# yhw-yhw/TalkSHOW

Hardware: AMD Instinct MI355X
Metric: generated SMPL-X frames/sec (10 s @ 30 fps clips), whole job (higher is better)
Workload: dtype f32; 1 GPU; BASELINE configs[1]: batch=32 x 10 s clips, body+hand VQ-VAE encode -> PixelCNN greedy decode -> VQ decode, 30 fps; batch_per_gpu=32, frames_per_clip=300, coalesce=8, streams=3

## Files before the change

include/talkshow_hip_debug.h:

```cpp
#ifndef TALKSHOW_HIP_DEBUG_H
#define TALKSHOW_HIP_DEBUG_H

#include "talkshow_hip.h"

#ifdef __cplusplus
extern "C" {
#endif

int ts_stream_create_cus(ts_ctx *ctx, int cu_first, int cu_count, void **out_stream);
int ts_debug_skinny_trace(unsigned long long *out, int max_records);
int ts_debug_clock_sample(unsigned long long *dev_out, int n, int window_us, void *stream);
int ts_debug_conv_bands(int M, int N, int groups, int *out4);
int ts_debug_split_tile(int bid, int MT, int NT, int gw, int *out2);
int ts_debug_tile_weights(const float *W, int N, int K, long ldw, int epi, int gateD, float *out);

int ts_op_conv1d_timed(ts_ctx *ctx, const float *x_dev, int B, int Lin, int Cin, const float *w_packed_dev,
                       const float *bias_dev, int Cout, int K, int tile, int iters, float *out_dev, float *ms_out,
                       void *stream);
int ts_op_conv1d_strided_timed(ts_ctx *ctx, const float *x_dev, int B, int Lin, int Cin, const float *w_packed_dev,
                               const float *bias_dev, int Cout, int K, int stride, int tile, int iters, float *out_dev,
                               float *ms_out, void *stream);

int ts_op_conv_taps48_timed(ts_ctx *ctx, const float *x_dev, int B, int T, int G, int ntap, const float *w_dev, const float *bias_dev,
                            const float *res_dev, int iters, float *out_dev, float *ms_out, void *stream);
// ... 118 lines not shown
int ts_debug_code_tables_plan(int V, int D, int B, int r, int j, int last_row, const char *knob_list, int64_t *out12);
int ts_debug_pixelcnn_tables(ts_pixelcnn *pix, int mode);
int64_t ts_debug_pixelcnn_work(ts_pixelcnn *pix, void *stream, int which, float *buf_dev, int64_t cap_floats, int put);
int ts_debug_code_table_stage(ts_pixelcnn *pix, int which, const int32_t *tok_dev, int B, const float *add1, const float *add2, const float *cls,
                              float *pre, float *out, float *q1, float *q0, void *stream);

int ts_debug_mixed_plan(const int32_t *hrows, int B, int max_counts, int32_t *active_out);

int ts_debug_rep_table(const ts_repeat *rep_host, int n_rep, int B, int V, int32_t *words_out);

int ts_op_vq_argmin_pair_masked(ts_ctx *ctx, const float *z_body_dev, const float *z_hand_dev, const int32_t *lens_dev, int B, int H_max,
                                const float *codebook_body_dev, const float *codebook_hand_dev, int ncode_body, int ncode_hand, int dim_body,
                                int dim_hand, int64_t *codes_dev, void *stream);
int ts_debug_vq_argmin_pair_masked(ts_ctx *ctx, const float *z_body_dev, const float *z_hand_dev, const int32_t *lens_dev, int B, int H_max,
                                   const float *codebook_body_dev, const float *codebook_hand_dev, int ncode_body, int ncode_hand,
                                   int dim_body, int dim_hand, int64_t *codes_dev, int form, int iters, void *stream);

int ts_debug_wino_lowering(int cin, int cout, int k, int stride, const char *knob_list, int B, int L, int *out5);
int ts_debug_wino_weights(const float *w, int cout, int cin, float *out);
int ts_debug_wino_transform(ts_ctx *ctx, int which, int nnet, int B, int L, int C, int act, const int32_t *lens_dev, int shr, int shl,
                            const void *const *ptrs, void *stream);
int ts_debug_wino_gemm(ts_ctx *ctx, int nnet, const float *V0, const float *V1, const float *U0, const float *U1, float *O0, float *O1, int M,
                       int C, void *stream);

int ts_debug_body_stream_plan(const int64_t *state4, int t, int flush, int enc_lowered, int64_t *out14);
int ts_debug_stream_stage_mfcc(const float *tail, const float *chunk, float *win, float *next, int B, int n_tail, int t, int cap, int Tw,
                               int next0, int n_next, void *stream);
int ts_debug_stream_emit(const int64_t *codes, int64_t *ring, int64_t *lat_body, int64_t *lat_hand, int B, int n, int A, int RC, int v0, int Hw,
                         void *stream);
int ts_debug_stream_keep_rows(const float *src, float *dst, int B, int R, int r0, int n, int W, void *stream);

int ts_debug_gather_rows(const float *table, int ld_table, int nrows, const int64_t *idx, long idx_stride, int M, int width, float *out,
                         int ldo, int L, const int32_t *lens, int len_shr, void *stream);
int ts_debug_pad_rows(const float *src, int lds, int c, float *dst, int ldd, int cpad, int B, int L, const int32_t *lens, void *stream);
int ts_debug_mask_rows(int64_t *codes, float *logprob, int B, int H, const int32_t *lens, void *stream);
int ts_debug_iota_i64(int64_t *dst, int n, int64_t first, void *stream);
int ts_debug_i64_to_i32(const int64_t *src, int32_t *dst, long n, void *stream);
int ts_debug_set_words3(uint64_t *dst, uint64_t a, uint64_t b, uint64_t c, void *stream);
int ts_debug_row_sqnorm(const float *e, int n, int dim, float *out, void *stream);

int ts_debug_skinny_chain(ts_ctx *ctx, int M, int K, int gate, int iters, int debug, float *us_out);

#ifdef __cplusplus
}
#endif
#endif
// ... 1 lines not shown
```

talkshow_amd/_lib.py:

```python
import ctypes as C
import os

import numpy as np
import torch

_HERE = os.path.dirname(os.path.abspath(__file__))
LIB_PATH = os.environ.get("TS_LIB_PATH") or os.path.join(_HERE, "lib", "libtalkshow_hip.so")

TS_SAMPLE_GREEDY, TS_SAMPLE_UNIFORMS, TS_SAMPLE_PHILOX, TS_TEACHER_FORCED = 0, 1, 2, 3


class TsTensor(C.Structure):
    _fields_ = [("name", C.c_char_p), ("data", C.POINTER(C.c_float)), ("ndim", C.c_int32), ("shape", C.c_int64 * 4)]


_vp, _i, _i64, _u64, _fp = C.c_void_p, C.c_int, C.c_int64, C.c_uint64, C.POINTER(C.c_float)


class TsSampling(C.Structure):
    _fields_ = [("temperature", C.c_float), ("top_p", C.c_float), ("top_k", C.c_int32), ("reserved", C.c_int32)]


_sp = C.POINTER(TsSampling)

# ... 154 lines not shown
    "ts_pixelcnn_generate_mixed": (_i, [_vp, _vp, _vp, C.POINTER(C.c_int32), _vp, _i, _i, _i, _vp, _u64, _vp, _vp, _vp]),
    "ts_vqvae_decode_pair_masked": (_i, [_vp, _vp, _vp, _vp, _vp, _i, _i, _vp, _vp]),
    "ts_debug_mixed_plan": (_i, [C.POINTER(C.c_int32), _i, _i, C.POINTER(C.c_int32)]),
    "ts_body_vq_infer": (_i, [_vp, _vp, _vp, _i, _i, _vp, _vp, _vp]),
    "ts_op_conv1d": (_i, [_vp, _vp, _i, _i, _i, _fp, _fp, _i, _i, _i, _i, _i, _i, _vp, _vp]),
    "ts_op_conv1d_timed": (_i, [_vp, _vp, _i, _i, _i, _vp, _vp, _i, _i, _i, _i, _vp, C.POINTER(C.c_float), _vp]),
    "ts_op_conv_taps48_timed": (_i, [_vp, _vp, _i, _i, _i, _i, _vp, _vp, _vp, _i, _vp, C.POINTER(C.c_float), _vp]),
    "ts_op_conv1d_strided_timed": (_i, [_vp, _vp, _i, _i, _i, _vp, _vp, _i, _i, _i, _i, _i, _vp, C.POINTER(C.c_float), _vp]),
    "ts_debug_pixelcnn_graphs": (_i, [_vp, _vp]),
    "ts_debug_code_tables_plan": (_i, [_i, _i, _i, _i, _i, _i, C.c_char_p, C.POINTER(_i64)]),
    "ts_debug_pixelcnn_tables": (_i, [_vp, _i]),
    "ts_debug_pixelcnn_work": (_i64, [_vp, _vp, _i, _vp, _i64, _i]),
    "ts_debug_code_table_stage": (_i, [_vp, _i, _vp, _i, _vp, _vp, _vp, _vp, _vp, _vp, _vp, _vp]),
    "ts_debug_conv_run": (_i, [_vp, C.POINTER(ConvProblem), _i, C.c_char_p, _i, C.POINTER(_i), _vp]),
    "ts_debug_conv_sk_plan": (_i, [_i, _i, _i, _i, C.POINTER(C.c_int)]),
    "ts_debug_conv_sk_run": (_i, [_i, _i, _i, _i, C.POINTER(C.c_int)]),
    "ts_debug_conv_sk_supported": (_i, []),
    "ts_pixelcnn_graph_captures": (C.c_long, [_vp, _vp]),
    "ts_pixelcnn_prepare": (_i, [_vp, _i, _i, _i, _vp]),
    "ts_debug_wino_lowering": (_i, [_i, _i, _i, _i, C.c_char_p, _i, _i, C.POINTER(_i)]),
    "ts_debug_wino_weights": (_i, [_vp, _i, _i, _vp]),
    "ts_debug_wino_transform": (_i, [_vp, _i, _i, _i, _i, _i, _i, _vp, _i, _i, C.POINTER(_vp), _vp]),
    "ts_debug_wino_gemm": (_i, [_vp, _i, _vp, _vp, _vp, _vp, _vp, _vp, _i, _i, _vp]),
    "ts_debug_conv_plan": (_i, [_i, _i, _i, _i, _i, C.POINTER(_i), _i, _i, C.c_char_p, C.POINTER(_i)]),
    "ts_debug_skinny_plan": (_i, [C.POINTER(_i), _i, C.c_char_p, C.POINTER(_i)]),
    "ts_debug_skinny_run": (_i, [_vp, C.POINTER(SkinnyProblem), _i, C.c_char_p, C.POINTER(_i), _vp]),
    "ts_debug_gate_act": (_i, [_vp, _vp, _vp, C.c_long, _vp]),
    "ts_debug_gelu": (_i, [_vp, _vp, C.c_long, _vp]),
    "ts_debug_attention": (_i, [_vp, _i, _i, _i, _i, C.c_float, _vp, _vp]),
    "ts_debug_layernorm_rows": (_i, [_vp, _i, C.c_long, _i, _vp, _vp, _vp, _i, _i, _vp, _i, _vp]),
    "ts_debug_lerp_ln": (_i, [_vp, _i, _i, _i, _vp, _vp, _vp, _vp]),
    "ts_debug_w2v_conv0": (_i, [_vp, _i, _i, _vp, _vp, _vp, _i, _vp, _vp]),
    "ts_debug_fill_id": (_i, [_vp, _i, _vp, _vp, _i, _vp, _i, _i, _i, _i, _vp]),
    "ts_debug_attention_mixed": (_i, [_vp, C.POINTER(C.c_int32), _vp, _i, _i, _i, _i, C.c_float, _vp, _vp]),
    "ts_debug_layernorm_rows_lens": (_i, [_vp, _i, _i, _i, _vp, _i, _vp, _vp, _vp, _i, _i, _vp, _i, _vp]),
    "ts_debug_lerp_ln_lens": (_i, [_vp, _i, _i, _i, _vp, _vp, _vp, _vp, _vp, _vp]),
    "ts_debug_w2v_conv0_lens": (_i, [_vp, _i, _i, _vp, _vp, _vp, _vp, _i, _vp, _vp]),
    "ts_debug_fill_id_lens": (_i, [_vp, _i, _vp, _vp, _i, _vp, _i, _i, _i, _i, _vp, _vp]),
    "ts_debug_face_mixed_grid": (_i, [C.POINTER(C.c_int32), _i, _i, C.POINTER(C.c_int32), _i]),
    "ts_debug_face_packed_layout": (_i, [C.POINTER(C.c_int32), C.POINTER(C.c_int32), _i, C.POINTER(_i64), C.POINTER(_i64), C.POINTER(_i64)]),
    "ts_debug_face_generate_mixed": (_i, [_vp, _vp, C.POINTER(C.c_int32), _vp, C.POINTER(C.c_int32), _vp, _i, _i, _i, _vp, _vp, _vp, _vp, _i]),
    "ts_debug_attention_packed": (_i, [_vp, C.POINTER(C.c_int32), _vp, _i, _i, _i, C.c_float, _vp, _vp]),
    "ts_debug_pack_rows": (_i, [_vp, C.POINTER(C.c_int32), _i, _i, _i, _vp, _vp]),
    "ts_debug_unpack_rows": (_i, [_vp, C.POINTER(C.c_int32), _vp, _i, _i, _i, _vp, _vp]),
    "ts_debug_w2v_conv0_packed": (_i, [_vp, _i, _i, C.POINTER(C.c_int32), _vp, _vp, _vp, _vp, _i, _vp, _vp]),
    "ts_debug_lerp_ln_packed": (_i, [_vp, _i, _i, C.POINTER(C.c_int32), _vp, _vp, _vp, _vp, _vp, _vp]),
# ... 605 lines not shown
```

talkshow_amd/csrc/api.cpp:

```cpp
#include <cstring>
#include <vector>
#include "host_common.h"
#include "conv_tile.h"
#include "skinny_desc.h"

using namespace ts;

namespace {
struct BodyWork {
    DevBuf feat;
    DevBuf lat[2];
    DevBuf given;
};
BodyWork &body_work(hipStream_t s) {
    static StreamWorks<BodyWork> works;
    return works.get(s);
}
}

namespace ts {
template <class Get>
static Knobs read_knobs(Get get) {
    Knobs v;
    auto num = [&](const char *name, int dflt) { const char *e = get(name); return e && e[0] ? std::atoi(e) : dflt; };
    v.conv_bands = num("TS_CONV_BANDS", 1) != 0;
    v.conv_ring = num("TS_CONV_RING", 9);
    v.conv_deal = num("TS_CONV_DEAL", 1) != 0;
    v.conv_ring_paired = num("TS_CONV_RING_PAIRED", 1) != 0;
    v.conv_taps48 = num("TS_CONV_TAPS48", 1) != 0;
    v.face_pack = num("TS_FACE_PACK", 0) != 0;
    v.conv_sk = num("TS_CONV_SK", 1);
    v.conv_wino = num("TS_CONV_WINO", -1);
    v.w2v_moments = num("TS_W2V_MOMENTS", 1) != 0;
    v.vq_lds = num("TS_VQ_LDS", 1) != 0;
    v.vq_pair = num("TS_VQ_PAIR", 1) != 0;
    v.split_xcd = num("TS_SPLIT_XCD", 8);
    v.prof_log = num("TS_PROF_LOG", 0) != 0;
    if (const char *e = get("TS_NO_GRAPH")) v.no_graph = e[0] && e[0] != '0';
    v.pix_defer_p = num("TS_PIX_DEFER_P", -1);
    v.pix_tables = num("TS_PIX_TABLES", -1);
    v.skinny_v = num("TS_SKINNY_V", 1);
    v.skinny_nt = num("TS_SKINNY_NT", 16);
    v.skinny_tiled = num("TS_SKINNY_TILED", 1) != 0;
    v.wide_min = num("TS_SKINNY_WIDE_MIN", 160);
    v.skinny_shape = num("TS_SKINNY_SHAPE", 0);
    v.skinny_trace = num("TS_SKINNY_TRACE", 0);
    v.wide_ablate = num("TS_SKINNY_WIDE_ABLATE", 0);
    v.wide_pair = num("TS_SKINNY_WIDE_PAIR", 1) != 0;
    return v;
}
const Knobs &knobs() {
    static const Knobs k = read_knobs([](const char *name) { return std::getenv(name); });
    return k;
}
static Knobs knobs_from_list(const char *list) {
// ... 1176 lines not shown
    std::memset(&w, 0, sizeof(w));
    w.nnet = nnet;
    w.B = B, w.L = L, w.J = (L + 3) / 4, w.C = C, w.act = act;
    w.lens = lens_dev, w.len_shr = shr, w.len_shl = shl;
    for (int i = 0; i < nnet; ++i) {
        const void *const *q = ptrs + 6 * i;
        w.x[i] = (const float *)q[0], w.V[i] = (float *)q[1], w.O[i] = (const float *)q[2], w.bias[i] = (const float *)q[3];
        w.res[i] = (const float *)q[4], w.y[i] = (float *)q[5];
    }
    MiscScope ms(ctx, (hipStream_t)stream);
    TS_HIP(ts::launch_wino(which, w, (hipStream_t)stream));
    return 0;
}

int ts_debug_wino_gemm(ts_ctx *ctx, int nnet, const float *V0, const float *V1, const float *U0, const float *U1, float *O0, float *O1, int M,
                       int C, void *stream) {
    if (!ctx || nnet < 1 || nnet > 2 || !V0 || !U0 || !O0 || (nnet == 2 && (!V1 || !U1 || !O1)) || M < 1 || C < 32 || C % 32)
        return fail("ts_debug_wino_gemm: bad argument");
    const float *V[2] = {V0, V1}, *U[2] = {U0, U1};
    float *O[2] = {O0, O1};
    return ts::run_wino_gemm(ctx, nnet, V, U, O, M, C, round_up(C, 128), (hipStream_t)stream);
}

int ts_debug_gather_rows(const float *table, int ld_table, int nrows, const int64_t *idx, long idx_stride, int M, int width, float *out,
                         int ldo, int L, const int32_t *lens, int len_shr, void *stream) {
    if (!table || !idx || !out || M < 1 || width < 1) return fail("ts_debug_gather_rows: bad argument");
    if (!lens && L == 0) TS_HIP(ts::launch_gather_rows(table, ld_table, nrows, idx, idx_stride, M, width, out, ldo, (hipStream_t)stream));
    else TS_HIP(ts::launch_gather_rows_masked(table, ld_table, nrows, idx, idx_stride, M, width, out, ldo, L, lens, len_shr, (hipStream_t)stream));
    return 0;
}
int ts_debug_pad_rows(const float *src, int lds, int c, float *dst, int ldd, int cpad, int B, int L, const int32_t *lens, void *stream) {
    if (!src || !dst || B < 1 || L < 1 || cpad < 1) return fail("ts_debug_pad_rows: bad argument");
    if (!lens) TS_HIP(ts::launch_pad_rows(src, lds, c, dst, ldd, cpad, (long)B * L, (hipStream_t)stream));
    else TS_HIP(ts::launch_pad_rows_masked(src, lds, c, dst, ldd, cpad, B, L, lens, (hipStream_t)stream));
    return 0;
}
int ts_debug_mask_rows(int64_t *codes, float *logprob, int B, int H, const int32_t *lens, void *stream) {
    if ((!codes && !logprob) || !lens || B < 1 || H < 1) return fail("ts_debug_mask_rows: bad argument");
    if (codes) TS_HIP(ts::launch_mask_codes(codes, B, H, lens, (hipStream_t)stream));
    if (logprob) TS_HIP(ts::launch_mask_logprob(logprob, B, H, lens, (hipStream_t)stream));
    return 0;
}
int ts_debug_iota_i64(int64_t *dst, int n, int64_t first, void *stream) {
    if (!dst || n < 1) return fail("ts_debug_iota_i64: bad argument");
    TS_HIP(ts::launch_iota_i64(dst, n, first, (hipStream_t)stream));
    return 0;
// ... 19 lines not shown
```

talkshow_amd/csrc/conv_wino.hip:

```cpp
#include "kernels.h"
#include "conv_tile.h"

namespace ts {

namespace {

__device__ __forceinline__ f32x4 ld4(const float *p) { return *reinterpret_cast<const f32x4 *>(p); }
__device__ __forceinline__ void st4(float *p, f32x4 v) { *reinterpret_cast<f32x4 *>(p) = v; }

__device__ __forceinline__ void wino_bt(const f32x4 (&d)[6], f32x4 (&v)[6]) {
#pragma clang fp contract(off)
    v[0] = (4.f * d[0] - 5.f * d[2]) + d[4];
    v[1] = ((d[3] - 4.f * d[1]) - 4.f * d[2]) + d[4];
    v[2] = ((4.f * d[1] - 4.f * d[2]) - d[3]) + d[4];
    v[3] = ((2.f * d[3] - 2.f * d[1]) - d[2]) + d[4];
    v[4] = ((2.f * d[1] - d[2]) - 2.f * d[3]) + d[4];
    v[5] = (4.f * d[1] - 5.f * d[3]) + d[5];
}

__device__ __forceinline__ f32x4 wino_at_row(const f32x4 (&m)[6], const int r) {
#pragma clang fp contract(off)
    if (r == 0) return (((m[0] + m[1]) + m[2]) + m[3]) + m[4];
    if (r == 1) return ((m[1] - m[2]) + 2.f * m[3]) - 2.f * m[4];
    if (r == 2) return ((m[1] + m[2]) + 4.f * m[3]) + 4.f * m[4];
// ... 3 lines not shown
__device__ __forceinline__ f32x4 wino_finish(f32x4 y, const f32x4 bias, const float *res, const int act) {
#pragma clang fp contract(off)
    f32x4 v = y + bias;
    if (res) v = v + ld4(res);
#pragma unroll
    for (int q = 0; q < 4; ++q) {
        float e = v[q];
        if (act == 1) e = e >= 0.f ? e : e * 0.2f;
        else if (act == 2) e = e > 0.f ? e : 0.f;
        else if (act == 3) e = gelu_fast(e);
        v[q] = e;
    }
    return v;
}

struct WinoItem {
    int net, b, j, c, Lb;
    long row;
    bool ok;
};
__device__ __forceinline__ WinoItem wino_item(const WinoParams &p) {
    WinoItem w;
    const int c4 = p.C >> 2;
    const long idx = (long)blockIdx.x * blockDim.x + threadIdx.x;
    w.net = blockIdx.y;
    w.row = idx / c4;
    w.c = (int)(idx - w.row * c4) << 2;
    w.ok = w.row < (long)p.B * p.J;
    w.b = (int)(w.row / p.J);
    w.j = (int)(w.row - (long)w.b * p.J);
    w.Lb = p.L;
    if (w.ok && p.lens) {
        const int l = (p.lens[w.b] >> p.len_shr) << p.len_shl;
        w.Lb = l < p.L ? l : p.L;
    }
    return w;
}

__device__ __forceinline__ void wino_load_tile(const float *O, const long comp_stride, const long row, const int C, const int c, f32x4 (&m)[6]) {
#pragma unroll
    for (int i = 0; i < 6; ++i) m[i] = ld4(O + i * comp_stride + row * C + c);
}

__global__ __launch_bounds__(256) void wino_in_kernel(const WinoParams p) {
    const WinoItem w = wino_item(p);
    if (!w.ok) return;
    const float *x = p.x[w.net] + (long)w.b * p.L * p.C + w.c;
    f32x4 d[6], v[6];
// ... 35 lines not shown
    const float *O = p.O[w.net];
    const f32x4 bias = ld4(p.bias[w.net] + w.c);
    const f32x4 zero{0.f, 0.f, 0.f, 0.f};
    f32x4 m[6], d[6], v[6];
    d[0] = zero;
    if (w.j > 0 && 4 * w.j - 1 < w.Lb) {
        wino_load_tile(O, cs, w.row - 1, p.C, w.c, m);
        d[0] = wino_finish(wino_at_row(m, 3), bias, nullptr, p.act);
    }
    wino_load_tile(O, cs, w.row, p.C, w.c, m);
#pragma unroll
    for (int r = 0; r < 4; ++r) d[1 + r] = 4 * w.j + r < w.Lb ? wino_finish(wino_at_row(m, r), bias, nullptr, p.act) : zero;
    d[5] = zero;
    if (w.j + 1 < p.J && 4 * w.j + 4 < w.Lb) {
        wino_load_tile(O, cs, w.row + 1, p.C, w.c, m);
        d[5] = wino_finish(wino_at_row(m, 0), bias, nullptr, p.act);
    }
    wino_bt(d, v);
    float *V = p.V[w.net] + w.row * p.C + w.c;
#pragma unroll
    for (int i = 0; i < 6; ++i) st4(V + i * cs, v[i]);
}

}

hipError_t launch_wino(int which, const WinoParams &p, hipStream_t stream) {
    if (p.nnet < 1 || p.nnet > 2 || p.B < 1 || p.L < 1 || p.C < 4 || (p.C & 3) || p.J != (p.L + 3) / 4 || p.act < 0 || p.act > 3 ||
        (p.lens && (p.len_shr < 0 || p.len_shl < 0)))
        return hipErrorInvalidValue;
    const long items = (long)p.B * p.J * (p.C >> 2);
    if (items + 255 >= (1l << 31)) return hipErrorInvalidValue;
    for (int n = 0; n < p.nnet; ++n) {
        const bool in = which == 0 ? p.x[n] && p.V[n] : which == 1 ? p.O[n] && p.bias[n] && p.y[n] : p.O[n] && p.bias[n] && p.V[n];
        if (!in) return hipErrorInvalidValue;
    }
    const dim3 grid((unsigned)((items + 255) / 256), p.nnet);
    if (which == 0) hipLaunchKernelGGL(wino_in_kernel, grid, dim3(256), 0, stream, p);
    else if (which == 1) hipLaunchKernelGGL(wino_out_kernel, grid, dim3(256), 0, stream, p);
    else if (which == 2) hipLaunchKernelGGL(wino_out_in_kernel, grid, dim3(256), 0, stream, p);
    else return hipErrorInvalidValue;
    return hipGetLastError();
}

void wino_transform_weights(const float *w, int cout, int cin, int npad, float *out) {
    static const double G[6][3] = {{1.0 / 4, 0, 0},          {-1.0 / 6, -1.0 / 6, -1.0 / 6}, {-1.0 / 6, 1.0 / 6, -1.0 / 6},
                                   {1.0 / 24, 1.0 / 12, 1.0 / 6}, {1.0 / 24, -1.0 / 12, 1.0 / 6}, {0, 0, 1}};
    for (int i = 0; i < 6; ++i)
        for (int o = 0; o < npad; ++o)
            for (int c = 0; c < cin; ++c) {
                double u = 0.0;
                if (o < cout) {
                    const float *g = w + ((size_t)o * cin + c) * 3;
                    u = G[i][0] * (double)g[0] + G[i][1] * (double)g[1] + G[i][2] * (double)g[2];
                }
                out[((size_t)i * npad + o) * cin + c] = (float)u;
            }
}

}
```

talkshow_amd/csrc/host_common.h:

```cpp
#pragma once
#include <hip/hip_runtime.h>

#include <cmath>
#include <cstring>
#include <map>
#include <atomic>
#include <memory>
#include <mutex>
#include <string>
#include <vector>

#include "../../include/talkshow_hip.h"
#include "../../include/talkshow_hip_debug.h"
#include "kernels.h"

namespace ts {

void set_error(const std::string &m);
inline int fail(const std::string &m) {
    set_error(m);
    return 1;
}

#define TS_HIP(expr)                                                                              \
// ... 173 lines not shown
};

struct ConvLayer {
    int kind = 0;
    int cin = 0, cin_pad = 0, cout = 0, cout_pad = 0, npad = 0, ktot = 0;
    int act = 0;
    int ngroups = 1, nseg = 0;
    ConvSeg segs[2][4];
    DevBuf w, bias;
    DevBuf wp;
    DevBuf wino;
    std::string name;
};

int pack_conv_layer(const StateDict &sd, const std::string &conv_key, const std::string &norm_key,
                    const std::string &res_key, int kind, int k, int cin, int cout, int act, ConvLayer *out);
int pack_linear_layer(const float *w, long ldw, const float *bias, int N, int K, ConvLayer *out);

int pack_conv_raw(const float *w, const float *bias, int cout, int cin, int K, const int *taps, int act, ConvLayer *out);

int conv_layer_params(const ConvLayer &layer, const float *x, int ldx, int B, int Lin, const float *res, int ldr,
                      float *out, int ldo, int out_col0, int n_store, ConvParams *p);

int run_wino_gemm(ts_ctx *ctx, int n, const float *const *V, const float *const *U, float *const *O, int M, int c, int npad, hipStream_t s);

int convnet_hidden(const ts_convnet *n);
int face_mixed_grid(const int32_t *frames, int B, int heads, std::vector<int> &work);
struct FacePacked {
    std::vector<int> feat_off, row0;
    long feat_rows = 0, rows = 0;
    int len[7] = {};
};
constexpr int FACE_FC_K[6] = {3, 3, 3, 3, 2, 2};
int face_packed_layout(const int32_t *ns, const int32_t *frames, int B, FacePacked *out);
int vqvae_in_dim(const ts_vqvae *v);
int vq_encode_pair_masked(ts_vqvae *vb, ts_vqvae *vh, const float *poses, int poses_ld, const int32_t *lens_dev, int B, int T_max, int64_t *codes,
                          int codes_H, float *z_body, float *z_hand, int form, hipStream_t s);

struct MixedPass {
    const int64_t *ids;
    const int32_t *lens_host, *lens_dev;
    int B, rows, mode;
    const float *uniforms;
    uint64_t seed;
    const int64_t *clip_index;
    int64_t *codes;
};
// ... 45 lines not shown
```

talkshow_amd/csrc/kernels.h:

```cpp
#pragma once
#include <hip/hip_runtime.h>
#include <stdint.h>

namespace ts {

struct Knobs;

struct ConvSeg {
    int d;
    int c0;
    int len;
    int ntap;
};

struct ConvGroup {
    const float *x;
    const float *w;
    const float *bias;
    const float *res;
    float *out;
    int out_col0;
    int nseg;
    ConvSeg seg[4];
};
// ... 89 lines not shown
    return true;
}

hipError_t launch_split_weight_planes(const float *w, float *planes, long rows, int K, hipStream_t stream);
double conv_gemm_flops(const ConvParams &p);

constexpr int WINO_MIN_C = 512;
inline bool wino_lowered(int kind, int k, int cin, int cout, int knob) {
    const bool geom = kind == 0 && k == 3 && cin == cout && cin % 32 == 0;
    return geom && knob != 0 && (knob == 1 || cout >= WINO_MIN_C);
}
struct WinoParams {
    int nnet;
    int B, L, J, C;
    int act;
    const int *lens;
    int len_shr, len_shl;
    const float *x[2];
    float *V[2];
    const float *O[2];
    const float *bias[2];
    const float *res[2];
    float *y[2];
};
hipError_t launch_wino(int which, const WinoParams &p, hipStream_t stream);
void wino_transform_weights(const float *w, int cout, int cin, int npad, float *out);

struct SkinnySeg {
    const float *base;
    const int *gidx;
    long row_stride;
    long gidx_stride;
    int row_shift;
    int len;
    int tiled_w;
};

enum { EPI_LINEAR = 0, EPI_GATE = 1 };
constexpr int SKINNY_MAX_SEG = 3;
constexpr int SKINNY_MAX_PROBLEMS = 6;

struct SkinnyParams {
    int M, N;
    int nseg, Ktot;
    SkinnySeg seg[SKINNY_MAX_SEG];
    const float *W;
// ... 126 lines not shown
    bool vq_lds = true;
    bool vq_pair = true;
    int conv_ring = 9;
    bool w2v_moments = true;
    int conv_sk = 1;
    bool face_pack = false;
    bool conv_taps48 = true;
    bool conv_ring_paired = true;
    bool conv_deal = true;
    int split_xcd = 8;
    bool prof_log = false;
    bool no_graph = false;
    int pix_defer_p = -1;
    int pix_tables = -1;
    int skinny_v = 1;
    int skinny_nt = 16;
    bool skinny_tiled = true;
    int wide_min = 160;
    int skinny_shape = 0;
    int skinny_trace = 0;
    bool wide_pair = true;
    int wide_ablate = 0;
    int conv_wino = -1;
};
const Knobs &knobs();

constexpr size_t CODE_TABLE_CAP_BYTES = (size_t)192 << 20;
constexpr int CODE_TABLE_MIN_CLIPS = 64;
struct CodeTablePlan {
    bool fits = false;
    int waves_v0 = 0, sets_v0 = 0, waves_hg = 0;
    size_t bytes_v0 = 0, bytes_hg = 0;
};
inline CodeTablePlan code_table_plan(int V, int D, const Knobs &k) {
    CodeTablePlan t;
    if (V < 1 || D < 32 || D % 32) return t;
    t.waves_v0 = code_table_waves(2 * D);
    t.sets_v0 = 1 + t.waves_v0 / 2;
    t.waves_hg = code_table_waves(D);
    t.bytes_v0 = (size_t)3 * t.sets_v0 * V * 4 * D * sizeof(float);
    t.bytes_hg = (size_t)V * 2 * D * sizeof(float);
    t.fits = k.skinny_nt != 32 && (size_t)V * 4 * D * sizeof(float) * 15 <= CODE_TABLE_CAP_BYTES;
    return t;
}
inline bool code_table_pass(bool built, int mode, int B) { return built && (mode > 0 || (mode < 0 && B >= CODE_TABLE_MIN_CLIPS)); }
inline bool code_table_v0_row(int r) { return r >= 1; }
// ... 178 lines not shown
```

talkshow_amd/csrc/models.cpp:

```cpp
#include <algorithm>
#include <cstdio>
#include "host_common.h"
#include "conv_tile.h"

namespace ts {

static thread_local std::string g_err;
void set_error(const std::string &m) { g_err = m; }
const char *last_error() { return g_err.c_str(); }

namespace {
std::mutex &scoped_mu() {
    static std::mutex m;
    return m;
}
std::vector<StreamScoped *> &scoped_all() {
    static std::vector<StreamScoped *> v;
    return v;
}
}
StreamScoped::StreamScoped() {
    std::lock_guard<std::mutex> g(scoped_mu());
    scoped_all().push_back(this);
}
// ... 242 lines not shown

int pack_linear_layer(const float *w, long ldw, const float *bias, int N, int K, ConvLayer *L) {
    L->kind = 0;
    L->cin = K;
    L->cin_pad = round_up(K, 32);
    L->cout = N;
    L->cout_pad = round_up(N, 32);
    L->npad = round_up(N, 128);
    L->act = 0;
    L->ngroups = 1;
    L->nseg = 1;
    L->ktot = L->cin_pad;
    L->segs[0][0] = ConvSeg{0, 0, L->cin_pad};
    std::vector<float> wp((size_t)L->npad * L->ktot, 0.f), bp(L->npad, 0.f);
    for (int o = 0; o < N; ++o) {
        for (int i = 0; i < K; ++i) wp[(size_t)o * L->ktot + i] = w[(long)o * ldw + i];
        if (bias) bp[o] = bias[o];
    }
    TS_TRY(L->w.upload(wp.data(), wp.size() * sizeof(float)));
    TS_TRY(L->bias.upload(bp.data(), bp.size() * sizeof(float)));
    return 0;
}

int run_wino_gemm(ts_ctx *ctx, int n, const float *const *V, const float *const *U, float *const *O, int M, int c, int npad, hipStream_t s) {
    auto dist = [](const float *a, const float *b) { return (long)((reinterpret_cast<intptr_t>(a) - reinterpret_cast<intptr_t>(b)) / (intptr_t)sizeof(float)); };
    ConvParams p;
    std::memset(&p, 0, sizeof(p));
    p.M = p.Lout = p.Lin = M;
    p.stride = 1;
    p.ldx = p.ldo = c;
    p.N = c;
    p.Ktot = c;
    p.ngroups = 6 * n;
    p.zdiv = 6;
    ConvGroup &g = p.g[0];
    g.x = V[0];
    g.w = U[0];
    g.out = O[0];
    g.nseg = 1;
    g.seg[0] = ConvSeg{0, 0, c, 1};
    p.x_zs1 = p.o_zs1 = (long)M * c;
    p.w_zs1 = (long)npad * c;
    if (n == 2) {
        p.x_zs0 = dist(V[1], V[0]);
        p.o_zs0 = dist(O[1], O[0]);
        p.w_zs0 = dist(U[1], U[0]);
    }
    const ConvPlan pl = plan_conv(p, 0, knobs(), false);
    const bool ring = pl.engine == ConvEngine::Reg && pl.bm == 128 && pl.bn == 128 && knobs().conv_ring > 0 && conv_gemm_ring_takes(p);
    return run_conv(ctx, p, ring ? 35 : 0, s);
}

int conv_layer_params(const ConvLayer &L, const float *x, int ldx, int B, int Lin, const float *res, int ldr,
                      float *out, int ldo, int out_col0, int n_store, ConvParams *p) {
    std::memset(p, 0, sizeof(*p));
    const int Lrows = L.kind == 1 ? Lin / 2 : Lin;
    p->M = B * Lrows;
    p->Lout = Lrows;
    p->Lin = Lin;
    p->stride = L.kind == 1 ? 2 : 1;
    p->ldx = ldx;
    p->ldr = ldr;
    p->N = n_store;
    p->Ktot = L.ktot;
// ... 116 lines not shown
                2 * L[0]->ngroups <= 4;
    if (same) {
        ConvParams &q = p[0];
        for (int g = 0; g < L[1]->ngroups; ++g) q.g[q.ngroups + g] = p[1].g[g];
        q.ngroups += L[1]->ngroups;
        return run_conv(ctx, q, 0, s);
    }
    for (int i = 0; i < n; ++i) TS_TRY(run_conv(ctx, p[i], 0, s));
    return 0;
}

int run_layer(ts_ctx *ctx, const ConvLayer &L, const float *x, int ldx, int B, int Lin, const float *res, int ldr,
              float *out, int ldo, int col0, int nstore, hipStream_t s, int *Lout, const LenMask *mk = nullptr) {
    const ConvLayer *Lp[1] = {&L};
    const float *xp[1] = {x}, *rp[1] = {res};
    float *op[1] = {out};
    return run_layer_n(ctx, 1, Lp, xp, ldx, B, Lin, rp, ldr, op, ldo, &col0, &nstore, s, Lout, mk);
}

size_t stack_wino_floats(const Stack &st, int c, int B, int L) {
    return st.tail.wino.p ? (size_t)6 * round_up(B * ((L + 3) / 4), 128) * c : 0;
}

int run_stack_wino(ts_ctx *ctx, int n, const Stack *const *st, Pool *const *pool, int cur, int c, int B, int L, hipStream_t s, int *out_idx,
                   const LenMask *mk) {
    WinoParams w;
    std::memset(&w, 0, sizeof(w));
    w.nnet = n;
    w.B = B, w.L = L, w.J = (L + 3) / 4, w.C = c;
    if (mk) w.lens = mk->lens, w.len_shr = mk->shr, w.len_shl = mk->shl;
    const int o = pool[0]->pick(cur), M = B * w.J;
    for (int i = 0; i < n; ++i) {
        if (pool[i]->wv.bytes < (size_t)6 * M * c * sizeof(float) || pool[i]->wo.bytes < (size_t)6 * M * c * sizeof(float))
            return fail("run_stack_wino: the Winograd arenas were not grown for this pass");
        w.x[i] = pool[i]->buf(cur);
        w.V[i] = pool[i]->wv.f();
        w.O[i] = pool[i]->wo.f();
        w.res[i] = pool[i]->buf(cur);
        w.y[i] = pool[i]->buf(o);
    }
    const ConvLayer *Lp[2];
    {
        MiscScope ms(ctx, s);
        TS_HIP(launch_wino(0, w, s));
    }
    const size_t nl = st[0]->layers.size();
    for (size_t k = 0; k <= nl; ++k) {
        for (int i = 0; i < n; ++i) {
            Lp[i] = k < nl ? st[i]->layers[k].get() : &st[i]->tail;
            w.bias[i] = Lp[i]->bias.f();
        }
        w.act = Lp[0]->act;
        const float *Vp[2] = {w.V[0], w.V[1]}, *Up[2] = {Lp[0]->wino.f(), n == 2 ? Lp[1]->wino.f() : nullptr};
        float *Op[2] = {pool[0]->wo.f(), n == 2 ? pool[1]->wo.f() : nullptr};
        TS_TRY(run_wino_gemm(ctx, n, Vp, Up, Op, M, c, Lp[0]->npad, s));
        MiscScope ms(ctx, s);
        TS_HIP(launch_wino(k < nl ? 2 : 1, w, s));
    }
    *out_idx = o;
    return 0;
}

int run_stack_n(ts_ctx *ctx, int n, const Stack *const *st, Pool *const *pool, int cur, int c, int B, int L, hipStream_t s,
                int *out_idx, const LenMask *mk = nullptr) {
    bool wino = true;
    for (int i = 0; i < n; ++i) {
        wino = wino && st[i]->tail.wino.p;
        for (const auto &l : st[i]->layers) wino = wino && l->wino.p;
    }
    if (wino) return run_stack_wino(ctx, n, st, pool, cur, c, B, L, s, out_idx, mk);
    int h = cur, tmp = 0;
    const int ns[2] = {c, c};
    const ConvLayer *Lp[2];
    const float *xp[2], *rp[2];
    float *op[2];
    for (size_t k = 0; k < st[0]->layers.size(); ++k) {
        const int o = pool[0]->pick(cur, h);
        for (int i = 0; i < n; ++i) { Lp[i] = st[i]->layers[k].get(); xp[i] = pool[i]->buf(h); op[i] = pool[i]->buf(o); }
        TS_TRY(run_layer_n(ctx, n, Lp, xp, c, B, L, nullptr, 0, op, c, nullptr, ns, s, &tmp, mk));
        h = o;
    }
    const int o = pool[0]->pick(cur, h);
    for (int i = 0; i < n; ++i) { Lp[i] = &st[i]->tail; xp[i] = pool[i]->buf(h); rp[i] = pool[i]->buf(cur); op[i] = pool[i]->buf(o); }
    TS_TRY(run_layer_n(ctx, n, Lp, xp, c, B, L, rp, c, op, c, nullptr, ns, s, &tmp, mk));
    *out_idx = o;
    return 0;
}

int run_trunk_n(int n, ts_convnet *const *net, const float *const *x, int x_ld, int B, int T, hipStream_t s, int *out_idx,
                int *H, const int *lens = nullptr) {
    if (T < 4) return fail("sequence too short: need T >= 4 frames");
    LenMask m0{lens, 0, 0}, m1{lens, 1, 0}, m2{lens, 2, 0};
    const LenMask *k0 = lens ? &m0 : nullptr, *k1 = lens ? &m1 : nullptr, *k2 = lens ? &m2 : nullptr;
// ... 47 lines not shown
    TS_TRY(run_layer_n(ctx, n, Lp, xp, hid / 2, B, L, nullptr, 0, op, hid, nullptr, ns, s, &L, k2));
    cur = o;
    for (int i = 0; i < n; ++i) Sp[i] = &net[i]->s3;
    TS_TRY(run_stack_n(ctx, n, Sp, pool, cur, hid, B, L, s, &o, k2));
    *out_idx = o;
    *H = L;
    return 0;
}

int run_trunk(ts_convnet *n, const float *x, int x_ld, int B, int T, hipStream_t s, int *out_idx, int *H, const int *lens = nullptr) {
    ts_convnet *np[1] = {n};
    const float *xp[1] = {x};
    return run_trunk_n(1, np, xp, x_ld, B, T, s, out_idx, H, lens);
}

}

struct ts_vqvae {
    ts_ctx *ctx = nullptr;
    int in_dim = 0, emb = 0, ncode = 0, hid = 0, nres = 0;
    ts_convnet enc;
    DevBuf codebook, code_sq;
    DevBuf aft_table;
    ConvLayer aft;
    Stack d1, d2, d3;
    ConvLayer up2, up3, project;
    struct Work {
        Pool pool;
        DevBuf z, lat;
        DevBuf pair;
    };
    StreamWorks<Work> works;
    Work &work(hipStream_t s) { return works.get(s); }
};

namespace {

int vq_encode_n(int n, ts_vqvae *const *vq, const float *const *poses, int poses_ld, int B, int T, float *const *z_out,
                int64_t *const *lat_out, float *const *q_out, hipStream_t s, int *Hout) {
    ts_ctx *ctx = vq[0]->ctx;
    int idx = 0, H = 0, tmp = 0;
    ts_convnet *nets[2];
    for (int i = 0; i < n; ++i) nets[i] = &vq[i]->enc;
    TS_TRY(run_trunk_n(n, nets, poses, poses_ld, B, T, s, &idx, &H));
    const ConvLayer *Lp[2];
    const float *xp[2];
// ... 42 lines not shown
    for (int i = 0; i < n; ++i) {
        if (vq[i]->hid != hid) return fail("paired VQ-VAEs must have the same width");
        pool[i] = &vq[i]->work(s).pool;
        TS_TRY(pool[i]->ensure((size_t)B * H * hid));
        TS_TRY(pool[i]->ensure_wino(std::max({stack_wino_floats(vq[i]->d1, hid, B, H), stack_wino_floats(vq[i]->d2, hid / 2, B, 2 * H),
                                              stack_wino_floats(vq[i]->d3, hid / 4, B, 4 * H)})));
        if (z && z[i]) {
            int tmp = 0;
            TS_TRY(run_layer(ctx, vq[i]->aft, z[i], vq[i]->emb, B, H, nullptr, 0, pool[i]->buf(0), hid, 0, hid, s, &tmp));
        } else {
            if (vq[i]->ncode == 0) return fail("this network has no codebook (auto-encoder): decode continuous latents");
            MiscScope ms(ctx, s);
            if (lens) TS_HIP(launch_gather_rows_masked(vq[i]->aft_table.f(), hid, vq[i]->ncode, lat[i], 1, B * H, hid, pool[i]->buf(0), hid, H, lens, 2, s));
            else TS_HIP(launch_gather_rows(vq[i]->aft_table.f(), hid, vq[i]->ncode, lat[i], 1, B * H, hid, pool[i]->buf(0), hid, s));
        }
    }
    int cur = 0, o = 0, L = H;
    const ConvLayer *Lp[2];
    const Stack *Sp[2];
    const float *xp[2];
    float *op[2];
    int ns[2];
    for (int i = 0; i < n; ++i) Sp[i] = &vq[i]->d1;
    TS_TRY(run_stack_n(ctx, n, Sp, pool, cur, hid, B, L, s, &o, k0));
    cur = o;
    o = pool[0]->pick(cur);
    for (int i = 0; i < n; ++i) { Lp[i] = &vq[i]->up2; xp[i] = pool[i]->buf(cur); op[i] = pool[i]->buf(o); ns[i] = hid / 2; }
    TS_TRY(run_layer_n(ctx, n, Lp, xp, hid, B, L, nullptr, 0, op, hid / 2, nullptr, ns, s, &L, k0));
    cur = o;
    for (int i = 0; i < n; ++i) Sp[i] = &vq[i]->d2;
    TS_TRY(run_stack_n(ctx, n, Sp, pool, cur, hid / 2, B, L, s, &o, k1));
    cur = o;
    o = pool[0]->pick(cur);
    for (int i = 0; i < n; ++i) { Lp[i] = &vq[i]->up3; xp[i] = pool[i]->buf(cur); op[i] = pool[i]->buf(o); ns[i] = hid / 4; }
    TS_TRY(run_layer_n(ctx, n, Lp, xp, hid / 2, B, L, nullptr, 0, op, hid / 4, nullptr, ns, s, &L, k1));
    cur = o;
    for (int i = 0; i < n; ++i) Sp[i] = &vq[i]->d3;
    TS_TRY(run_stack_n(ctx, n, Sp, pool, cur, hid / 4, B, L, s, &o, k2));
    int tmp = 0;
    for (int i = 0; i < n; ++i)
        TS_TRY(run_layer(ctx, vq[i]->project, pool[i]->buf(o), hid / 4, B, L, nullptr, 0, out, out_ld, col0[i], vq[i]->in_dim, s, &tmp, k2));
    return 0;
}

int vq_decode_impl(ts_vqvae *vq, const int64_t *lat, int B, int H, float *out, int out_ld, int col0, hipStream_t s) {
    ts_vqvae *vp[1] = {vq};
    const int64_t *lp[1] = {lat};
// ... 138 lines not shown
    vq->ctx = ctx;
    vq->in_dim = in_dim;
    vq->emb = emb;
    vq->ncode = ncode;
    vq->hid = hid;
    vq->nres = nres;
    TS_TRY(pack_trunk(ctx, sd, "encoder.", in_dim, hid, nres, &vq->enc));
    vq->enc.has_pre_vq = true;
    TS_TRY(pack_conv_layer(sd, "encoder.pre_vq_conv", "", "", 0, 1, hid, emb, 0, &vq->enc.pre_vq));
    TS_TRY(pack_conv_layer(sd, "decoder.aft_vq_conv", "", "", 0, 1, emb, hid, 0, &vq->aft));
    if (ncode > 0) {
        const float *cb = sd.get("vq_layer.embeddings", {ncode, emb});
        if (!cb) return 1;
        TS_TRY(vq->codebook.upload(cb, (size_t)ncode * emb * sizeof(float)));
        TS_TRY(vq->code_sq.ensure((size_t)ncode * sizeof(float)));
        TS_HIP(launch_row_sqnorm(vq->codebook.f(), ncode, emb, vq->code_sq.f(), 0));
        TS_TRY(vq->aft_table.ensure((size_t)ncode * hid * sizeof(float)));
        ConvParams p;
        conv_layer_params(vq->aft, vq->codebook.f(), emb, 1, ncode, nullptr, 0, vq->aft_table.f(), hid, 0, hid, &p);
        TS_HIP(launch_conv_gemm(p, 0, 0));
        TS_HIP(hipStreamSynchronize(0));
    }
    TS_TRY(pack_stack(sd, "decoder._dec_1", hid, nres, &vq->d1));
    TS_TRY(pack_conv_layer(sd, "decoder._up_2.conv", "decoder._up_2.norm", "decoder._up_2.residual_layer", 2, 4, hid,
                           hid / 2, 1, &vq->up2));
    TS_TRY(pack_stack(sd, "decoder._dec_2", hid / 2, nres, &vq->d2));
    TS_TRY(pack_conv_layer(sd, "decoder._up_3.conv", "decoder._up_3.norm", "decoder._up_3.residual_layer", 2, 4,
                           hid / 2, hid / 4, 1, &vq->up3));
    TS_TRY(pack_stack(sd, "decoder._dec_3", hid / 4, nres, &vq->d3));
    TS_TRY(pack_conv_layer(sd, "decoder.project", "", "", 0, 1, hid / 4, in_dim, 0, &vq->project));
    *out = vq.release();
    return 0;
}
void ts_vqvae_destroy(ts_vqvae *vq) { delete vq; }

int ts_vqvae_encode(ts_vqvae *vq, const float *poses, int B, int T, float *z, int64_t *lat, float *q, void *stream) {
    if (!vq || !poses) return fail("ts_vqvae_encode: null argument");
    if (vq->ncode > 0 && !lat) return fail("ts_vqvae_encode: latents_dev is required for a network with a codebook");
    if (vq->ncode == 0 && (!z || lat || q)) return fail("ts_vqvae_encode: an auto-encoder (num_embeddings = 0) produces z only");
    int H = 0;
    return vq_encode_impl(vq, poses, 0, B, T, z, lat, q, (hipStream_t)stream, &H);
}

int ts_vqvae_decode(ts_vqvae *vq, const int64_t *lat, int B, int H, float *out, int out_ld, int col0, void *stream) {
    if (!vq || !lat || !out) return fail("ts_vqvae_decode: null argument");
    if (out_ld < col0 + vq->in_dim) return fail("ts_vqvae_decode: out_ld too small");
// ... 86 lines not shown
    if (!vb || !vh || !poses || !lens) return fail("ts_body_vq_infer_mixed: null argument");
    if (!codes && !recon) return fail("ts_body_vq_infer_mixed: nothing to produce");
    if (B < 1) return fail("ts_body_vq_infer_mixed: bad shape");
    hipStream_t s = (hipStream_t)stream;
    const int H = T_max / 4;
    if (!codes) {
        ts_vqvae::Work &wk = vb->work(s);
        TS_TRY(wk.pair.ensure((size_t)B * (H + 1) * 2 * sizeof(int64_t)));
        codes = static_cast<int64_t *>(wk.pair.p);
    }
    TS_TRY(vq_encode_pair_masked(vb, vh, poses, vb->in_dim + vh->in_dim, lens, B, T_max, codes, H, nullptr, nullptr, 0, s));
    if (!recon) return 0;
    ts_vqvae *vqs[2] = {vb, vh};
    int64_t *lp[2];
    for (int k = 0; k < 2; ++k) {
        ts_vqvae::Work &wk = vqs[k]->work(s);
        TS_TRY(wk.lat.ensure((size_t)B * (H + 1) * sizeof(int64_t)));
        lp[k] = static_cast<int64_t *>(wk.lat.p);
        TS_HIP(hipMemcpy2DAsync(lp[k], sizeof(int64_t), codes + k, 2 * sizeof(int64_t), sizeof(int64_t), (size_t)B * H, hipMemcpyDeviceToDevice, s));
    }
    return ts_vqvae_decode_pair_masked(vb, vh, lp[0], lp[1], lens, B, H, recon, s);
}

}
```

Baseline: 2.029 million frames/s.

## Precompute Winograd-domain decoder tables per code and deal wino blocks across XCDs

At load time, each VQ codebook entry's aft-conv output is pushed through the first decoder residual layer's Winograd weight transform. The result is stored as per-code tables. At decode time a new kernel gathers those rows by latent code and applies the input transform directly, skipping the first Winograd input transform plus GEMM of the d1 stack. Separately, wino kernels can remap block indices round-robin across 8 groups (the 'deal' path) to spread work across dies. The trade-off is extra device memory for the tables and reliance on linearity of the transform and GEMM for exactness, with possible fp rounding differences.

After: 2.087 million frames/s, median of 6. 2.9% higher.

```diff
diff --git a/include/talkshow_hip_debug.h b/include/talkshow_hip_debug.h
--- a/include/talkshow_hip_debug.h
+++ b/include/talkshow_hip_debug.h
@@ -164,6 +164,9 @@
                             const void *const *ptrs, void *stream);
 int ts_debug_wino_gemm(ts_ctx *ctx, int nnet, const float *V0, const float *V1, const float *U0, const float *U1, float *O0, float *O1, int M,
                        int C, void *stream);
+int ts_debug_wino_codes(ts_ctx *ctx, int nnet, int B, int L, int C, const int32_t *lens_dev, int shr, int shl, const int64_t *codes0,
+                        const int64_t *codes1, const float *T0, const float *T1, int ncode0, int ncode1, float *O0, float *O1, void *stream);
+int ts_debug_vqvae_dec_tables(ts_vqvae *vq, float *tables, float *aft_table, float *u, const float **tables_dev);
 
 int ts_debug_body_stream_plan(const int64_t *state4, int t, int flush, int enc_lowered, int64_t *out14);
 int ts_debug_stream_stage_mfcc(const float *tail, const float *chunk, float *win, float *next, int B, int n_tail, int t, int cap, int Tw,
diff --git a/talkshow_amd/_lib.py b/talkshow_amd/_lib.py
--- a/talkshow_amd/_lib.py
+++ b/talkshow_amd/_lib.py
@@ -200,6 +200,8 @@
     "ts_debug_wino_weights": (_i, [_vp, _i, _i, _vp]),
     "ts_debug_wino_transform": (_i, [_vp, _i, _i, _i, _i, _i, _i, _vp, _i, _i, C.POINTER(_vp), _vp]),
     "ts_debug_wino_gemm": (_i, [_vp, _i, _vp, _vp, _vp, _vp, _vp, _vp, _i, _i, _vp]),
+    "ts_debug_wino_codes": (_i, [_vp, _i, _i, _i, _i, _vp, _i, _i, _vp, _vp, _vp, _vp, _i, _i, _vp, _vp, _vp]),
+    "ts_debug_vqvae_dec_tables": (_i, [_vp, _vp, _vp, _vp, C.POINTER(_vp)]),
     "ts_debug_conv_plan": (_i, [_i, _i, _i, _i, _i, C.POINTER(_i), _i, _i, C.c_char_p, C.POINTER(_i)]),
     "ts_debug_skinny_plan": (_i, [C.POINTER(_i), _i, C.c_char_p, C.POINTER(_i)]),
     "ts_debug_skinny_run": (_i, [_vp, C.POINTER(SkinnyProblem), _i, C.c_char_p, C.POINTER(_i), _vp]),
diff --git a/talkshow_amd/csrc/api.cpp b/talkshow_amd/csrc/api.cpp
--- a/talkshow_amd/csrc/api.cpp
+++ b/talkshow_amd/csrc/api.cpp
@@ -31,6 +31,8 @@
     v.face_pack = num("TS_FACE_PACK", 0) != 0;
     v.conv_sk = num("TS_CONV_SK", 1);
     v.conv_wino = num("TS_CONV_WINO", -1);
+    v.vq_dec_tables = num("TS_VQ_DEC_TABLES", -1);
+    v.wino_deal = num("TS_WINO_DEAL", 1) != 0;
     v.w2v_moments = num("TS_W2V_MOMENTS", 1) != 0;
     v.vq_lds = num("TS_VQ_LDS", 1) != 0;
     v.vq_pair = num("TS_VQ_PAIR", 1) != 0;
@@ -1253,6 +1255,20 @@
     return ts::run_wino_gemm(ctx, nnet, V, U, O, M, C, round_up(C, 128), (hipStream_t)stream);
 }
 
+int ts_debug_wino_codes(ts_ctx *ctx, int nnet, int B, int L, int C, const int32_t *lens_dev, int shr, int shl, const int64_t *codes0,
+                        const int64_t *codes1, const float *T0, const float *T1, int ncode0, int ncode1, float *O0, float *O1, void *stream) {
+    if (!ctx || nnet < 1 || nnet > 2) return fail("ts_debug_wino_codes: bad argument");
+    ts::WinoParams w;
+    std::memset(&w, 0, sizeof(w));
+    w.nnet = nnet;
+    w.B = B, w.L = L, w.J = (L + 3) / 4, w.C = C;
+    w.lens = lens_dev, w.len_shr = shr, w.len_shl = shl;
+    w.codes[0] = codes0, w.codes[1] = codes1, w.T[0] = T0, w.T[1] = T1, w.ncode[0] = ncode0, w.ncode[1] = ncode1, w.Ow[0] = O0, w.Ow[1] = O1;
+    MiscScope ms(ctx, (hipStream_t)stream);
+    TS_HIP(ts::launch_wino(3, w, (hipStream_t)stream));
+    return 0;
+}
+
 int ts_debug_gather_rows(const float *table, int ld_table, int nrows, const int64_t *idx, long idx_stride, int M, int width, float *out,
                          int ldo, int L, const int32_t *lens, int len_shr, void *stream) {
     if (!table || !idx || !out || M < 1 || width < 1) return fail("ts_debug_gather_rows: bad argument");
diff --git a/talkshow_amd/csrc/conv_wino.hip b/talkshow_amd/csrc/conv_wino.hip
--- a/talkshow_amd/csrc/conv_wino.hip
+++ b/talkshow_amd/csrc/conv_wino.hip
@@ -49,8 +49,15 @@
 __device__ __forceinline__ WinoItem wino_item(const WinoParams &p) {
     WinoItem w;
     const int c4 = p.C >> 2;
-    const long idx = (long)blockIdx.x * blockDim.x + threadIdx.x;
+    unsigned bx = blockIdx.x;
     w.net = blockIdx.y;
+    if (p.deal) {
+        const unsigned total = gridDim.x, q = total >> 3, r = total & 7, x = bx & 7;
+        const unsigned g = x * q + (x < r ? x : r) + (bx >> 3);
+        w.net = g >= (unsigned)p.deal;
+        bx = g - (w.net ? p.deal : 0);
+    }
+    const long idx = (long)bx * blockDim.x + threadIdx.x;
     w.row = idx / c4;
     w.c = (int)(idx - w.row * c4) << 2;
     w.ok = w.row < (long)p.B * p.J;
@@ -132,6 +139,38 @@
     for (int i = 0; i < 6; ++i) st4(V + i * cs, v[i]);
 }
 
+__global__ __launch_bounds__(256) void wino_codes_kernel(const WinoParams p) {
+#pragma clang fp contract(off)
+    const WinoItem w = wino_item(p);
+    if (!w.ok) return;
+    const int ncode = p.ncode[w.net];
+    const int64_t *codes = p.codes[w.net] + (long)w.b * p.L;
+    long off[6];
+#pragma unroll
+    for (int k = 0; k < 6; ++k) {
+        const int t = 4 * w.j - 1 + k;
+        off[k] = -1;
+        if (t >= 0 && t < w.Lb) {
+            const int64_t r = codes[t];
+            if (r >= 0 && r < ncode) off[k] = (long)r * p.C + w.c;
+        }
+    }
+    const float *T = p.T[w.net];
+    const long ts = (long)ncode * p.C;
+    auto row = [&](const int i, const int k) { return off[k] >= 0 ? ld4(T + i * ts + off[k]) : f32x4{0.f, 0.f, 0.f, 0.f}; };
+    f32x4 v[6];
+    v[0] = (4.f * row(0, 0) - 5.f * row(0, 2)) + row(0, 4);
+    v[1] = ((row(1, 3) - 4.f * row(1, 1)) - 4.f * row(1, 2)) + row(1, 4);
+    v[2] = ((4.f * row(2, 1) - 4.f * row(2, 2)) - row(2, 3)) + row(2, 4);
+    v[3] = ((2.f * row(3, 3) - 2.f * row(3, 1)) - row(3, 2)) + row(3, 4);
+    v[4] = ((2.f * row(4, 1) - row(4, 2)) - 2.f * row(4, 3)) + row(4, 4);
+    v[5] = (4.f * row(5, 1) - 5.f * row(5, 3)) + row(5, 5);
+    const long cs = (long)p.B * p.J * p.C;
+    float *O = p.Ow[w.net] + w.row * p.C + w.c;
+#pragma unroll
+    for (int i = 0; i < 6; ++i) st4(O + i * cs, v[i]);
+}
+
 }
 
 hipError_t launch_wino(int which, const WinoParams &p, hipStream_t stream) {
@@ -141,13 +180,20 @@
     const long items = (long)p.B * p.J * (p.C >> 2);
     if (items + 255 >= (1l << 31)) return hipErrorInvalidValue;
     for (int n = 0; n < p.nnet; ++n) {
-        const bool in = which == 0 ? p.x[n] && p.V[n] : which == 1 ? p.O[n] && p.bias[n] && p.y[n] : p.O[n] && p.bias[n] && p.V[n];
+        const bool in = which == 0   ? p.x[n] && p.V[n]
+                        : which == 1 ? p.O[n] && p.bias[n] && p.y[n]
+                        : which == 2 ? p.O[n] && p.bias[n] && p.V[n]
+                                     : p.codes[n] && p.T[n] && p.Ow[n] && p.ncode[n] > 0;
         if (!in) return hipErrorInvalidValue;
     }
-    const dim3 grid((unsigned)((items + 255) / 256), p.nnet);
-    if (which == 0) hipLaunchKernelGGL(wino_in_kernel, grid, dim3(256), 0, stream, p);
-    else if (which == 1) hipLaunchKernelGGL(wino_out_kernel, grid, dim3(256), 0, stream, p);
-    else if (which == 2) hipLaunchKernelGGL(wino_out_in_kernel, grid, dim3(256), 0, stream, p);
+    const unsigned nb = (unsigned)((items + 255) / 256);
+    WinoParams q = p;
+    q.deal = knobs().wino_deal && conv_sk_supported() ? (int)nb : 0;
+    const dim3 grid = q.deal ? dim3(nb * p.nnet) : dim3(nb, p.nnet);
+    if (which == 0) hipLaunchKernelGGL(wino_in_kernel, grid, dim3(256), 0, stream, q);
+    else if (which == 1) hipLaunchKernelGGL(wino_out_kernel, grid, dim3(256), 0, stream, q);
+    else if (which == 2) hipLaunchKernelGGL(wino_out_in_kernel, grid, dim3(256), 0, stream, q);
+    else if (which == 3) hipLaunchKernelGGL(wino_codes_kernel, grid, dim3(256), 0, stream, q);
     else return hipErrorInvalidValue;
     return hipGetLastError();
 }
diff --git a/talkshow_amd/csrc/host_common.h b/talkshow_amd/csrc/host_common.h
--- a/talkshow_amd/csrc/host_common.h
+++ b/talkshow_amd/csrc/host_common.h
@@ -219,7 +219,8 @@
 int conv_layer_params(const ConvLayer &layer, const float *x, int ldx, int B, int Lin, const float *res, int ldr,
                       float *out, int ldo, int out_col0, int n_store, ConvParams *p);
 
-int run_wino_gemm(ts_ctx *ctx, int n, const float *const *V, const float *const *U, float *const *O, int M, int c, int npad, hipStream_t s);
+int run_wino_gemm(ts_ctx *ctx, int n, const float *const *V, const float *const *U, float *const *O, int M, int c, int npad, hipStream_t s,
+                  bool one_v = false);
 
 int convnet_hidden(const ts_convnet *n);
 int face_mixed_grid(const int32_t *frames, int B, int heads, std::vector<int> &work);
diff --git a/talkshow_amd/csrc/kernels.h b/talkshow_amd/csrc/kernels.h
--- a/talkshow_amd/csrc/kernels.h
+++ b/talkshow_amd/csrc/kernels.h
@@ -135,6 +135,11 @@
     const float *bias[2];
     const float *res[2];
     float *y[2];
+    const int64_t *codes[2];
+    const float *T[2];
+    int ncode[2];
+    float *Ow[2];
+    int deal;
 };
 hipError_t launch_wino(int which, const WinoParams &p, hipStream_t stream);
 void wino_transform_weights(const float *w, int cout, int cin, int npad, float *out);
@@ -307,6 +312,8 @@
     bool wide_pair = true;
     int wide_ablate = 0;
     int conv_wino = -1;
+    bool wino_deal = true;
+    int vq_dec_tables = -1;
 };
 const Knobs &knobs();
 
diff --git a/talkshow_amd/csrc/models.cpp b/talkshow_amd/csrc/models.cpp
--- a/talkshow_amd/csrc/models.cpp
+++ b/talkshow_amd/csrc/models.cpp
@@ -288,7 +288,8 @@
     return 0;
 }
 
-int run_wino_gemm(ts_ctx *ctx, int n, const float *const *V, const float *const *U, float *const *O, int M, int c, int npad, hipStream_t s) {
+int run_wino_gemm(ts_ctx *ctx, int n, const float *const *V, const float *const *U, float *const *O, int M, int c, int npad, hipStream_t s,
+                  bool one_v) {
     auto dist = [](const float *a, const float *b) { return (long)((reinterpret_cast<intptr_t>(a) - reinterpret_cast<intptr_t>(b)) / (intptr_t)sizeof(float)); };
     ConvParams p;
     std::memset(&p, 0, sizeof(p));
@@ -305,7 +306,8 @@
     g.out = O[0];
     g.nseg = 1;
     g.seg[0] = ConvSeg{0, 0, c, 1};
-    p.x_zs1 = p.o_zs1 = (long)M * c;
+    p.o_zs1 = (long)M * c;
+    p.x_zs1 = one_v ? 0 : p.o_zs1;
     p.w_zs1 = (long)npad * c;
     if (n == 2) {
         p.x_zs0 = dist(V[1], V[0]);
@@ -468,8 +470,14 @@
     return st.tail.wino.p ? (size_t)6 * round_up(B * ((L + 3) / 4), 128) * c : 0;
 }
 
+struct CodeSrc {
+    const int64_t *codes[2];
+    const float *T[2];
+    int ncode[2];
+};
+
 int run_stack_wino(ts_ctx *ctx, int n, const Stack *const *st, Pool *const *pool, int cur, int c, int B, int L, hipStream_t s, int *out_idx,
-                   const LenMask *mk) {
+                   const LenMask *mk, const CodeSrc *src) {
     WinoParams w;
     std::memset(&w, 0, sizeof(w));
     w.nnet = n;
@@ -484,11 +492,12 @@
         w.O[i] = pool[i]->wo.f();
         w.res[i] = pool[i]->buf(cur);
         w.y[i] = pool[i]->buf(o);
+        if (src) w.codes[i] = src->codes[i], w.T[i] = src->T[i], w.ncode[i] = src->ncode[i], w.Ow[i] = pool[i]->wo.f();
     }
     const ConvLayer *Lp[2];
     {
         MiscScope ms(ctx, s);
-        TS_HIP(launch_wino(0, w, s));
+        TS_HIP(launch_wino(src ? 3 : 0, w, s));
     }
     const size_t nl = st[0]->layers.size();
     for (size_t k = 0; k <= nl; ++k) {
@@ -499,7 +508,7 @@
         w.act = Lp[0]->act;
         const float *Vp[2] = {w.V[0], w.V[1]}, *Up[2] = {Lp[0]->wino.f(), n == 2 ? Lp[1]->wino.f() : nullptr};
         float *Op[2] = {pool[0]->wo.f(), n == 2 ? pool[1]->wo.f() : nullptr};
-        TS_TRY(run_wino_gemm(ctx, n, Vp, Up, Op, M, c, Lp[0]->npad, s));
+        if (k > 0 || !src) TS_TRY(run_wino_gemm(ctx, n, Vp, Up, Op, M, c, Lp[0]->npad, s));
         MiscScope ms(ctx, s);
         TS_HIP(launch_wino(k < nl ? 2 : 1, w, s));
     }
@@ -508,13 +517,14 @@
 }
 
 int run_stack_n(ts_ctx *ctx, int n, const Stack *const *st, Pool *const *pool, int cur, int c, int B, int L, hipStream_t s,
-                int *out_idx, const LenMask *mk = nullptr) {
+                int *out_idx, const LenMask *mk = nullptr, const CodeSrc *src = nullptr) {
     bool wino = true;
     for (int i = 0; i < n; ++i) {
         wino = wino && st[i]->tail.wino.p;
         for (const auto &l : st[i]->layers) wino = wino && l->wino.p;
     }
-    if (wino) return run_stack_wino(ctx, n, st, pool, cur, c, B, L, s, out_idx, mk);
+    if (wino) return run_stack_wino(ctx, n, st, pool, cur, c, B, L, s, out_idx, mk, src);
+    if (src) return fail("run_stack_n: code tables given for a stack that is not lowered");
     int h = cur, tmp = 0;
     const int ns[2] = {c, c};
     const ConvLayer *Lp[2];
@@ -608,6 +618,7 @@
     ts_convnet enc;
     DevBuf codebook, code_sq;
     DevBuf aft_table;
+    DevBuf dec_tables;
     ConvLayer aft;
     Stack d1, d2, d3;
     ConvLayer up2, up3, project;
@@ -696,7 +707,14 @@
     float *op[2];
     int ns[2];
     for (int i = 0; i < n; ++i) Sp[i] = &vq[i]->d1;
-    TS_TRY(run_stack_n(ctx, n, Sp, pool, cur, hid, B, L, s, &o, k0));
+    CodeSrc src;
+    std::memset(&src, 0, sizeof(src));
+    bool tables = true;
+    for (int i = 0; i < n; ++i) {
+        tables = tables && lat && lat[i] && !(z && z[i]) && vq[i]->dec_tables.p;
+        src.codes[i] = lat ? lat[i] : nullptr, src.T[i] = vq[i]->dec_tables.f(), src.ncode[i] = vq[i]->ncode;
+    }
+    TS_TRY(run_stack_n(ctx, n, Sp, pool, cur, hid, B, L, s, &o, k0, tables ? &src : nullptr));
     cur = o;
     o = pool[0]->pick(cur);
     for (int i = 0; i < n; ++i) { Lp[i] = &vq[i]->up2; xp[i] = pool[i]->buf(cur); op[i] = pool[i]->buf(o); ns[i] = hid / 2; }
@@ -881,6 +899,16 @@
         TS_HIP(hipStreamSynchronize(0));
     }
     TS_TRY(pack_stack(sd, "decoder._dec_1", hid, nres, &vq->d1));
+    {
+        const ConvLayer &l0 = vq->d1.layers.empty() ? vq->d1.tail : *vq->d1.layers[0];
+        if (ncode > 0 && l0.wino.p && knobs().vq_dec_tables != 0) {
+            TS_TRY(vq->dec_tables.ensure(((size_t)5 * ncode + round_up(ncode, 128)) * hid * sizeof(float)));
+            const float *Vp[1] = {vq->aft_table.f()}, *Up[1] = {l0.wino.f()};
+            float *Op[1] = {vq->dec_tables.f()};
+            TS_TRY(run_wino_gemm(ctx, 1, Vp, Up, Op, ncode, hid, l0.npad, 0, true));
+            TS_HIP(hipStreamSynchronize(0));
+        }
+    }
     TS_TRY(pack_conv_layer(sd, "decoder._up_2.conv", "decoder._up_2.norm", "decoder._up_2.residual_layer", 2, 4, hid,
                            hid / 2, 1, &vq->up2));
     TS_TRY(pack_stack(sd, "decoder._dec_2", hid / 2, nres, &vq->d2));
@@ -1013,4 +1041,16 @@
     return ts_vqvae_decode_pair_masked(vb, vh, lp[0], lp[1], lens, B, H, recon, s);
 }
 
-}
+int ts_debug_vqvae_dec_tables(ts_vqvae *vq, float *tables, float *aft_table, float *u, const float **tables_dev) {
+    if (!vq) return -1;
+    if (!vq->dec_tables.p) return 0;
+    const ConvLayer &l0 = vq->d1.layers.empty() ? vq->d1.tail : *vq->d1.layers[0];
+    const size_t t = (size_t)vq->ncode * vq->hid * sizeof(float);
+    if (tables && copy_and_wait(tables, vq->dec_tables.p, 6 * t, hipMemcpyDeviceToHost) != hipSuccess) return -1;
+    if (aft_table && copy_and_wait(aft_table, vq->aft_table.p, t, hipMemcpyDeviceToHost) != hipSuccess) return -1;
+    if (u && copy_and_wait(u, l0.wino.p, (size_t)6 * l0.npad * vq->hid * sizeof(float), hipMemcpyDeviceToHost) != hipSuccess) return -1;
+    if (tables_dev) *tables_dev = vq->dec_tables.f();
+    return 1;
+}
+
+}
```
